# antopio26/quadruped-gym

Hardware: AMD Instinct MI355X
Metric: env_steps_per_sec (higher is better)
Workload: dtype f32

## Files before the change

### quadruped-gym_amd/csrc/qg_kernel_link.hip

```cpp
#define QGK_LINK_ENVS 4
#include "qg_po_dev.h"

typedef const __attribute__((address_space(1))) char *lk_gcbytes;
typedef __attribute__((address_space(1))) char *lk_gbytes;
template <class T> DEV T lk_ld(const T *base, unsigned byte_off) { return *(const __attribute__((address_space(1))) T *)((lk_gcbytes)base + byte_off); }
template <class T> DEV void lk_st(T *base, unsigned byte_off, T v) { *(__attribute__((address_space(1))) T *)((lk_gbytes)base + byte_off) = v; }

template <int CTRL> DEV float dpp_any(float x) {
    return __builtin_bit_cast(float, __builtin_amdgcn_mov_dpp(__builtin_bit_cast(int, x), CTRL, 0xF, 0xF, true));
}
DEV float env_sum(float x) {
#pragma clang fp contract(off)
    x += dpp_any<0xB1>(x);
    x += dpp_any<0x4E>(x);
    x += dpp_any<0x141>(x);
    x += dpp_any<0x140>(x);
    return x;
}
DEV V3 env_sum(V3 a) { return v3(env_sum(a.x), env_sum(a.y), env_sum(a.z)); }
#define QG_T_HM(d, s, bm) "v_add_f32_dpp %[" d "], %[" s "], %[" s "] row_half_mirror row_mask:0xf bank_mask:" bm "\n\t"
#define QG_T_ROR(d, s, bm) "v_add_f32_dpp %[" d "], %[" s "], %[" s "] row_ror:8 row_mask:0xf bank_mask:" bm "\n\t"
#define QG_T_QP(d, qp) "v_add_f32_dpp %[" d "], %[" d "], %[" d "] quad_perm:" qp " row_mask:0xf bank_mask:0xf\n\t"
#define QG_T_L1(g) QG_T_HM("a" g, "a" g, "0x5") QG_T_HM("c" g, "c" g, "0x5") QG_T_HM("a" g, "b" g, "0xa") QG_T_HM("c" g, "d" g, "0xa")
#define QG_T_L2(g) QG_T_ROR("a" g, "a" g, "0x3") QG_T_ROR("a" g, "c" g, "0xc")
#define QG_T_Q1(g) QG_T_QP("a" g, "[1,0,3,2]")
#define QG_T_Q2(g) QG_T_QP("a" g, "[2,3,0,1]")
#define QG_T_OUT(g, v) [a##g] "+v"(v[4 * g]), [c##g] "+v"(v[4 * g + 2])
#define QG_T_IN(g, v) [b##g] "v"(v[4 * g + 1]), [d##g] "v"(v[4 * g + 3])
DEV void env_sum_banked16(float (&v)[16]) {
    asm("s_nop 1\n\t" QG_T_L1("0") QG_T_L1("1") QG_T_L1("2") QG_T_L1("3") QG_T_L2("0") QG_T_L2("1") QG_T_L2("2") QG_T_L2("3")
        QG_T_Q1("0") QG_T_Q1("1") QG_T_Q1("2") QG_T_Q1("3") QG_T_Q2("0") QG_T_Q2("1") QG_T_Q2("2") QG_T_Q2("3") "s_nop 1"
        : QG_T_OUT(0, v), QG_T_OUT(1, v), QG_T_OUT(2, v), QG_T_OUT(3, v)
        : QG_T_IN(0, v), QG_T_IN(1, v), QG_T_IN(2, v), QG_T_IN(3, v));
}
DEV void env_sum_banked12(float (&v)[12]) {
    asm("s_nop 1\n\t" QG_T_L1("0") QG_T_L1("1") QG_T_L1("2") QG_T_L2("0") QG_T_L2("1") QG_T_L2("2")
        QG_T_Q1("0") QG_T_Q1("1") QG_T_Q1("2") QG_T_Q2("0") QG_T_Q2("1") QG_T_Q2("2") "s_nop 1"
        : QG_T_OUT(0, v), QG_T_OUT(1, v), QG_T_OUT(2, v)
        : QG_T_IN(0, v), QG_T_IN(1, v), QG_T_IN(2, v));
}
template <int K> DEV float banked_sum(float r) { return dpp_any<0x150 + 4 * K>(r); }
DEV float leg_suffix(float x) {
#pragma clang fp contract(off)
    x += dpp_any<0xF9>(x);
    x += dpp_any<0xFE>(x);
    return x;
}
DEV float leg_bcast0(float x) { return dpp_any<0x00>(x); }
DEV float leg_bcast1(float x) { return dpp_any<0x55>(x); }
DEV float leg_bcast2(float x) { return dpp_any<0xAA>(x); }

DEV float leg_prefix(float x) {
#pragma clang fp contract(off)
    x += dpp_any<0xD3>(x);
    x += dpp_any<0x4F>(x);
    return x;
}
DEV V3 leg_prefix(V3 a) { return v3(leg_prefix(a.x), leg_prefix(a.y), leg_prefix(a.z)); }

struct LinkRegs {
    float mass, ipos[3], inertia[6], cp[QGK_CP_LINK][3];
    f2 cp2[QGK_CP_LINK / 2][3];
    float lo, hi, damping, armature, kp, kv, gear, force_lo, force_hi, act_decay;
    float cpF[3];
    float ml;
    float fb[8];
};
struct HingeLane { float q, qd, act, u, sn, cs; };
struct KXfrcLink { KWrench w; V3 c0; };

DEV float sel3(int r, float a, float b, float c) { return r == 0 ? a : (r == 1 ? b : c); }
DEV V3 sel3(int r, V3 a, V3 b, V3 c) { return v3(sel3(r, a.x, b.x, c.x), sel3(r, a.y, b.y, c.y), sel3(r, a.z, b.z, c.z)); }

template <bool BAKED, bool DYN = false>
DEV void substep_link(const KModel &C, float cm, float sm, int r, bool lead_env, BaseState &B, HingeLane &J, const LinkRegs &K,
                      bool want_sensors, float *__restrict__ row, int kleg, float &zaxis_z, const KDyn &D = KDyn{}, bool xon = false,
                      const KXfrcLink &X = KXfrcLink{}) {
    using namespace pk3;
    const float h = C.h;
    const BaseCtx bc = pk3::base_prelude_unit(C, B);
    const V3 nb = bc.n;
    if (want_sensors) {
        zaxis_z = bc.cz.z;
        if (r < 3) row[3 * kleg + r] = J.q;
        if (lead_env) {
            row[15] = B.wb.x; row[16] = B.wb.y; row[17] = B.wb.z;
            row[18] = B.pw.x; row[19] = B.pw.y; row[20] = B.pw.z;
            row[21] = B.vw.x; row[22] = B.vw.y; row[23] = B.vw.z;
            row[24] = bc.cx.x; row[25] = bc.cx.y; row[26] = bc.cx.z;
            row[27] = bc.cz.x; row[28] = bc.cz.y; row[29] = bc.cz.z;
            row[30] = bc.vb.x; row[31] = bc.vb.y; row[32] = bc.vb.z;
        }
    }
    const int rr = r < 2 ? r : 2;
    const float snj[3] = {leg_bcast0(J.sn), leg_bcast1(J.sn), leg_bcast2(J.sn)};
    const float csj[3] = {leg_bcast0(J.cs), leg_bcast1(J.cs), leg_bcast2(J.cs)};
    Fr E[3];
    V3 p[3];
    SV S[3];
    {
        Fr Ep = {v3(BAKED ? cm : 1.f, BAKED ? sm : 0.f, 0.f), v3(BAKED ? -sm : 0.f, BAKED ? cm : 1.f, 0.f), v3(0.f, 0.f, 1.f)};
        V3 pp = v3(0.f, 0.f, 0.f);
#pragma unroll
        for (int i = 0; i < 3; ++i) {
            const KLink &L = link_of<BAKED>(C, kleg, i);
            const float sn = snj[i], cs = csj[i];
            p[i] = pp + rot(Ep, ld3(L.pos));
            V3 tx = fma3(L.Q[0], Ep.ex, fma3(L.Q[3], Ep.ey, L.Q[6] * Ep.ez));
            V3 ty = fma3(L.Q[1], Ep.ex, fma3(L.Q[4], Ep.ey, L.Q[7] * Ep.ez));
            V3 tz = fma3(L.Q[2], Ep.ex, fma3(L.Q[5], Ep.ey, L.Q[8] * Ep.ez));
            E[i].ex = fma3(cs, tx, sn * ty);
            E[i].ey = fma3(cs, ty, (-sn) * tx);
            E[i].ez = tz;
// ... 29 lines not shown
        V3 uz = fma3(K.inertia[4], E.ex, fma3(K.inertia[5], E.ey, K.inertia[2] * E.ez));
        float hc = dot(Bi.h, c);
        const f2 uxp = {ux.x, ux.y}, uyp = {uy.x, uy.y}, uzp = {uz.x, uz.y}, hp = {Bi.h.x, Bi.h.y}, cp2 = {c.x, c.y};
        const f2 d2 = __builtin_elementwise_fma(uxp, f2{E.ex.x, E.ex.y}, __builtin_elementwise_fma(uyp, f2{E.ey.x, E.ey.y}, uzp * f2{E.ez.x, E.ez.y}))
                      + f2{hc, hc} - hp * cp2;
        const f2 o2 = __builtin_elementwise_fma(uxp, f2{E.ex.z, E.ex.z}, __builtin_elementwise_fma(uyp, f2{E.ey.z, E.ey.z}, uzp * f2{E.ez.z, E.ez.z}))
                      - hp * f2{c.z, c.z};
        Bi.I.xx = d2.x; Bi.I.yy = d2.y; Bi.I.xz = o2.x; Bi.I.yz = o2.y;
        Bi.I.zz = fmaf(ux.z, E.ex.z, fmaf(uy.z, E.ey.z, uz.z * E.ez.z)) + hc - Bi.h.z * c.z;
        Bi.I.xy = fmaf(ux.x, E.ex.y, fmaf(uy.x, E.ey.y, uz.x * E.ez.y)) - Bi.h.x * c.y;
    }
    SV f;
    {
        SV Iv = mul(Bi, vp), Ia = mul(Bi, ap);
        f.a = cross_add(vp.l, Iv.l, cross_add(vp.a, Iv.a, Ia.a));
        f.l = cross_add(vp.a, Iv.l, Ia.l);
    }
    Sym6 A = sym6_of(Bi);
    {
        const float zo = B.pw.z + dot(nb, pp);
        V3 nl = rotT(Ep, nb);
        float wsum = 0.f;
        V3 s = v3(0.f, 0.f, 0.f);
        const float zb = C.contact_margin - zo;
        if constexpr (BAKED) {
            static_assert(QGK_CP_LINK % 2 == 0, "sample points are taken in pairs");
            f2 w2 = {0.f, 0.f};
            V3T<f2> s2 = v3<f2>(w2, w2, w2);
            const V3T<f2> nl2 = v3<f2>(f2{nl.x, nl.x}, f2{nl.y, nl.y}, f2{nl.z, nl.z});
            const f2 zb2 = {zb, zb};
#pragma unroll
            for (int i = 0; i < QGK_CP_LINK / 2; ++i) contact_point(v3<f2>(K.cp2[i][0], K.cp2[i][1], K.cp2[i][2]), nl2, zb2, w2, s2);
            wsum = w2.x + w2.y;
            s = v3(s2.x.x + s2.x.y, s2.y.x + s2.y.y, s2.z.x + s2.z.y);
        } else {
#pragma unroll
            for (int i = 0; i < QGK_CP_LINK; ++i) contact_point(v3(K.cp[i][0], K.cp[i][1], K.cp[i][2]), nl, zb, wsum, s);
        }
        wsum *= K.ml;
        SV fe;
        ContactDampT<float> cd;
        if constexpr (DYN) pk3::contact_eval(wsum, s, Ep, pp, nb, vp, D.kc, D.cc, C.contact_inv_ramp, D.mu, h, fe, cd);
        else pk3::contact_eval(wsum, s, Ep, pp, nb, vp, C.contact_k, C.contact_c, C.contact_inv_ramp, C.contact_mu, h, fe, cd);
        f.a = f.a - fe.a;
        f.l = f.l - fe.l;
        pk3::add_contact_damping(A, cd.mc, cd.w, cd.P, nb);
    }
    SV xw = {};
    if constexpr (DYN) {
        if (xon) {
            xw = xfrc_spatial(bc, X.w, r < 3 ? cl : X.c0);
            f.a = fma3(-K.ml, xw.a, f.a);
            f.l = fma3(-K.ml, xw.l, f.l);
        }
    }
    float wsumF = 0.f;
    V3 sF = v3(0.f, 0.f, 0.f);
    contact_point(v3(K.cpF[0], K.cpF[1], K.cpF[2]), nb, C.contact_margin - B.pw.z, wsumF, sF);
    wsumF *= K.ml; sF = K.ml * sF;
    Sym6 Ic;
    SV fc;
    Ic.AA.xx = leg_suffix(A.AA.xx); Ic.AA.yy = leg_suffix(A.AA.yy); Ic.AA.zz = leg_suffix(A.AA.zz);
    Ic.AA.xy = leg_suffix(A.AA.xy); Ic.AA.xz = leg_suffix(A.AA.xz); Ic.AA.yz = leg_suffix(A.AA.yz);
    Ic.AL.r0 = v3(leg_suffix(A.AL.r0.x), leg_suffix(A.AL.r0.y), leg_suffix(A.AL.r0.z));
    Ic.AL.r1 = v3(leg_suffix(A.AL.r1.x), leg_suffix(A.AL.r1.y), leg_suffix(A.AL.r1.z));
    Ic.AL.r2 = v3(leg_suffix(A.AL.r2.x), leg_suffix(A.AL.r2.y), leg_suffix(A.AL.r2.z));
    Ic.LL.xx = leg_suffix(A.LL.xx); Ic.LL.yy = leg_suffix(A.LL.yy); Ic.LL.zz = leg_suffix(A.LL.zz);
    Ic.LL.xy = leg_suffix(A.LL.xy); Ic.LL.xz = leg_suffix(A.LL.xz); Ic.LL.yz = leg_suffix(A.LL.yz);
    fc.a = v3(leg_suffix(f.a.x), leg_suffix(f.a.y), leg_suffix(f.a.z));
    fc.l = v3(leg_suffix(f.l.x), leg_suffix(f.l.y), leg_suffix(f.l.z));
    const SV F = mul(Ic, So);
    const float Hc0 = dot(S[0], F), Hc1 = dot(S[1], F);
    const float Hown = dot(So, F);
    const float tb = dot(So, fc);
    float Hd_o, b_o;
    {
        const float q = J.q, qd = J.qd, act = J.act;
        float force = K.kp * (act - K.gear * q) - (K.kv * K.gear) * qd;
        const bool clamped = force <= K.force_lo || force >= K.force_hi;
        force = fminf(fmaxf(force, K.force_lo), K.force_hi);
        float dimp = K.damping + (clamped ? 0.f : K.kv * K.gear * K.gear);
        float tau = K.gear * force - K.damping * qd;
        const float below = K.lo - q, above = q - K.hi;
        const float pen = fmaxf(fmaxf(below, above), 0.f);
        const float bl = C.limit_b * fminf(pen * C.limit_inv_ramp, 1.f);
        const float sg = below > above ? 1.f : -1.f;
        const float sqd = sg * qd;
        const float spring = C.limit_k * pen;
        const float tq = spring - bl * sqd;
        const bool leaving = tq < 0.f;
        tau = fmaf(sg, fmaxf(tq, 0.f), tau);
        dimp = dimp + (leaving ? spring * rcp(sqd) : bl);
        Hd_o = Hown + K.armature + h * dimp;
        b_o = tau - tb;
    }
    const float H00 = leg_bcast0(Hd_o), H01 = leg_bcast1(Hc0), H11 = leg_bcast1(Hd_o);
    const float H02 = leg_bcast2(Hc0), H12 = leg_bcast2(Hc1), H22 = leg_bcast2(Hd_o);
    const float b0 = leg_bcast0(b_o), b1 = leg_bcast1(b_o), b2 = leg_bcast2(b_o);
    const float id0 = rcp(H00);
    const float l10 = H01 * id0, l20 = H02 * id0;
    const float d1 = fmaf(-l10, H01, H11), id1 = rcp(d1);
    const float t21 = fmaf(-l20, H01, H12);
    const float l21 = t21 * id1;
    const float d2 = fmaf(-l21, t21, fmaf(-l20, H02, H22)), id2 = rcp(d2);
    const float y0 = b0, y1 = fmaf(-l10, y0, b1), y2 = fmaf(-l21, y1, fmaf(-l20, y0, b2));
    float z[6] = {F.a.x, F.a.y, F.a.z, F.l.x, F.l.y, F.l.z};
    {
        const float nc0 = r == 1 ? -l10 : (r == 2 ? -l20 : 0.f), nc1 = r == 2 ? -l21 : 0.f;
#pragma unroll
        for (int i = 0; i < 6; ++i) z[i] = fmaf(leg_bcast0(z[i]), nc0, z[i]);
#pragma unroll
        for (int i = 0; i < 6; ++i) z[i] = fmaf(leg_bcast1(z[i]), nc1, z[i]);
    }
    const float idr = sel3(rr, id0, id1, id2), yr = sel3(rr, y0, y1, y2);
    const f2 P = {z[0], z[1]}, L = {z[3], z[4]}, Z = {z[2], z[5]};
    const f2 idr2 = {idr, idr};
    const f2 WP = idr2 * P, WL = idr2 * L, WZ = idr2 * Z;
    Sym6 Cn;
    {
        const f2 Zlo = {Z.x, Z.x}, Zhi = {Z.y, Z.y};
        const f2 WPlo = {WP.x, WP.x}, WPhi = {WP.y, WP.y}, WZlo = {WZ.x, WZ.x};
        const f2 aa0 = __builtin_elementwise_fma(-WP, P, f2{A.AA.xx, A.AA.yy});
        const f2 aa1 = __builtin_elementwise_fma(-WP, Zlo, f2{A.AA.xz, A.AA.yz});
        Cn.AA.xx = aa0.x; Cn.AA.yy = aa0.y; Cn.AA.xz = aa1.x; Cn.AA.yz = aa1.y;
        Cn.AA.xy = fmaf(-WP.x, P.y, A.AA.xy); Cn.AA.zz = fmaf(-WZ.x, Z.x, A.AA.zz);
        const f2 c0 = __builtin_elementwise_fma(-WPlo, L, f2{A.AL.r0.x, A.AL.r0.y});
        const f2 c1 = __builtin_elementwise_fma(-WPhi, L, f2{A.AL.r1.x, A.AL.r1.y});
        const f2 c2 = __builtin_elementwise_fma(-WZlo, L, f2{A.AL.r2.x, A.AL.r2.y});
        const f2 c3 = __builtin_elementwise_fma(-WP, Zhi, f2{A.AL.r0.z, A.AL.r1.z});
        Cn.AL.r0 = v3(c0.x, c0.y, c3.x);
        Cn.AL.r1 = v3(c1.x, c1.y, c3.y);
        Cn.AL.r2 = v3(c2.x, c2.y, fmaf(-WZ.x, Z.y, A.AL.r2.z));
        const f2 l0 = __builtin_elementwise_fma(-WL, L, f2{A.LL.xx, A.LL.yy});
        const f2 l1 = __builtin_elementwise_fma(-WL, Zhi, f2{A.LL.xz, A.LL.yz});
        Cn.LL.xx = l0.x; Cn.LL.yy = l0.y; Cn.LL.xz = l1.x; Cn.LL.yz = l1.y;
        Cn.LL.xy = fmaf(-WL.x, L.y, A.LL.xy); Cn.LL.zz = fmaf(-WZ.y, Z.y, A.LL.zz);
    }
    if constexpr (DYN) {
        if (xon) {
            f.a = fma3(K.ml - 1.f, xw.a, f.a);
            f.l = fma3(K.ml - 1.f, xw.l, f.l);
        }
    }
    const f2 nyr = {-yr, -yr};
    const f2 rh0 = __builtin_elementwise_fma(nyr, WP, f2{-f.a.x, -f.a.y}), rh1 = __builtin_elementwise_fma(nyr, WL, f2{-f.l.x, -f.l.y}),
             rh2 = __builtin_elementwise_fma(nyr, WZ, f2{-f.a.z, -f.l.z});
    SV rhn = {v3(rh0.x, rh0.y, rh2.x), v3(rh1.x, rh1.y, rh2.y)};
    float x6[6];
    {
        SV p0;
        Sym6 Ic0;
        pk3::frame_body_pk<DYN>(C, bc, h, p0, Ic0, D);
        if constexpr (BAKED) {
            Ic0.AA.xx = K.fb[0]; Ic0.AA.yy = K.fb[1]; Ic0.AA.zz = K.fb[2]; Ic0.LL.xx = K.fb[3]; Ic0.LL.yy = K.fb[4]; Ic0.LL.zz = K.fb[5];
            Ic0.AL.r0.y = K.fb[6]; Ic0.AL.r1.x = K.fb[7];
        }
        float t16[16] = {Cn.AA.xx, Cn.AA.yy, Cn.AA.zz, Cn.AA.xy, Cn.AA.xz, Cn.AA.yz, Cn.AL.r0.x, Cn.AL.r0.y,
                         Cn.AL.r0.z, Cn.AL.r1.x, Cn.AL.r1.y, Cn.AL.r1.z, Cn.AL.r2.x, Cn.AL.r2.y, Cn.AL.r2.z, wsumF};
        float t12[12] = {Cn.LL.xx, Cn.LL.yy, Cn.LL.zz, Cn.LL.xy, Cn.LL.xz, Cn.LL.yz, rhn.a.x, rhn.a.y, rhn.a.z, rhn.l.x, rhn.l.y, rhn.l.z};
        env_sum_banked16(t16);
        env_sum_banked12(t12);
        Ic0.AA.xx += banked_sum<0>(t16[0]); Ic0.AA.yy += banked_sum<1>(t16[0]); Ic0.AA.zz += banked_sum<2>(t16[0]); Ic0.AA.xy += banked_sum<3>(t16[0]);
        Ic0.AA.xz += banked_sum<0>(t16[4]); Ic0.AA.yz += banked_sum<1>(t16[4]); Ic0.AL.r0.x += banked_sum<2>(t16[4]); Ic0.AL.r0.y += banked_sum<3>(t16[4]);
        Ic0.AL.r0.z += banked_sum<0>(t16[8]); Ic0.AL.r1.x += banked_sum<1>(t16[8]); Ic0.AL.r1.y += banked_sum<2>(t16[8]); Ic0.AL.r1.z += banked_sum<3>(t16[8]);
        Ic0.AL.r2.x += banked_sum<0>(t16[12]); Ic0.AL.r2.y += banked_sum<1>(t16[12]); Ic0.AL.r2.z += banked_sum<2>(t16[12]);
        wsumF = banked_sum<3>(t16[12]);
        Ic0.LL.xx += banked_sum<0>(t12[0]); Ic0.LL.yy += banked_sum<1>(t12[0]); Ic0.LL.zz += banked_sum<2>(t12[0]); Ic0.LL.xy += banked_sum<3>(t12[0]);
        Ic0.LL.xz += banked_sum<0>(t12[4]); Ic0.LL.yz += banked_sum<1>(t12[4]);
        SV b = {v3(banked_sum<2>(t12[4]) - p0.a.x, banked_sum<3>(t12[4]) - p0.a.y, banked_sum<0>(t12[8]) - p0.a.z),
                v3(banked_sum<1>(t12[8]) - p0.l.x, banked_sum<2>(t12[8]) - p0.l.y, banked_sum<3>(t12[8]) - p0.l.z)};
        if (__any(wsumF > 0.f)) {
            sF = env_sum(sF);
            Fr E0 = {v3(1.f, 0.f, 0.f), v3(0.f, 1.f, 0.f), v3(0.f, 0.f, 1.f)};
            SV fe;
            if constexpr (DYN) contact_finish(wsumF, sF, E0, v3(0.f, 0.f, 0.f), bc.n, bc.V0, D.kc, D.cc, C.contact_inv_ramp, D.mu, h, fe, Ic0);
            else contact_finish(wsumF, sF, E0, v3(0.f, 0.f, 0.f), bc.n, bc.V0, C.contact_k, C.contact_c, C.contact_inv_ramp, C.contact_mu, h, fe, Ic0);
            b.a = b.a + fe.a;
            b.l = b.l + fe.l;
        }
        pk3::base_solve(Ic0, b, x6);
    }
    const V3 wdot = v3(x6[0], x6[1], x6[2]);
    const V3 acl = v3(x6[3], x6[4], x6[5]);
    if (want_sensors && lead_env) {
        row[12] = acl.x - bc.gb.x; row[13] = acl.y - bc.gb.y; row[14] = acl.z - bc.gb.z;
    }
    {
        const float g_o = fmaf(F.a.x, x6[0], fmaf(F.a.y, x6[1], fmaf(F.a.z, x6[2], fmaf(F.l.x, x6[3], fmaf(F.l.y, x6[4], F.l.z * x6[5])))));
        const float r0 = b0 - leg_bcast0(g_o), r1 = b1 - leg_bcast1(g_o), r2 = b2 - leg_bcast2(g_o);
        const float yy0 = r0, yy1 = fmaf(-l10, yy0, r1), yy2 = fmaf(-l21, yy1, fmaf(-l20, yy0, r2));
        const float qdd2 = yy2 * id2;
        const float qdd1 = fmaf(-l21, qdd2, yy1 * id1);
        const float qdd0 = fmaf(-l20, qdd2, fmaf(-l10, qdd1, yy0 * id0));
        J.qd = fmaf(h, sel3(rr, qdd0, qdd1, qdd2), J.qd);
        J.q = fmaf(h, J.qd, J.q);
        hinge_advance(h * J.qd, J.sn, J.cs);
        J.act = fmaf(J.u - J.act, K.act_decay, J.act);
    }
    pk3::base_integrate_unit(bc, h, wdot, acl, B);
}

#define QGK_LINK_WAVES 4
template <bool WALK = false, bool PO = false, bool BAKED = true, bool HELP = false, bool DYN = false>
__global__ __launch_bounds__(QGK_WAVE * QGK_LINK_WAVES * (HELP ? 2 : 1), 1) void qg_step_kernel_link(const KModel *__restrict__ Mp, const KTask *__restrict__ T, KStepArgs P,
                                                                                  const typename WalkArgT<WALK>::type WK,
                                                                                  const typename PoArgT<PO>::type PK) {
    static_assert(WALK || !PO, "the observation pack rides on the walking task layer");
    static_assert(WALK || !HELP, "the helper waves carry the walking task layer's estimator");
    static_assert(!DYN || (!BAKED && !HELP), "per-env dynamics: the table-driven variants");
    static_assert(QGK_LINK_ENVS * QGK_LINK_WAVES == QG_PO_ENVS && QGK_WAVE * QGK_LINK_WAVES == QG_PO_THREADS, "workgroup layout of qg_po_dev.h");
    __shared__ float tile_all[QGK_LINK_WAVES][QGK_LINK_ENVS * 35];
    __shared__ KModel smodel;
    QG_STAGE_MODEL(C, BAKED, smodel, Mp, QGK_WAVE * QGK_LINK_WAVES * (HELP ? 2 : 1));
    QG_TASK_REGS(Tk, T);
    QG_MARK(0);
    const int lane = threadIdx.x & (QGK_WAVE - 1);
    const int wave = (threadIdx.x >> 6) & (QGK_LINK_WAVES - 1);
    const bool helper = HELP && (threadIdx.x >> 6) >= QGK_LINK_WAVES;
    float *tile = tile_all[wave];
    const int r = lane & 3;
    const int k = (lane >> 2) & 3;
    const int el = lane >> 4;
    const int env0 = (blockIdx.x * QGK_LINK_WAVES + wave) * QGK_LINK_ENVS;
    const int n = P.n;
    const bool live = env0 + el < n;
    const int env = live ? env0 + el : n - 1;
    const bool lead_env = (lane & 15) == 0;
    const float cm = (k == 0) ? 1.f : (k == 2) ? -1.f : 0.f;
    const float sm = (k == 1) ? 1.f : (k == 3) ? -1.f : 0.f;

    constexpr bool RWDH = HELP && !PO;
    __shared__ float s_est[HELP ? QGK_LINK_WAVES : 1][QGK_WAVE][2];
// ... 150 lines not shown
            if constexpr (!HELP) walk_estimator_finish_n<1>(WK.P, WK.S, n, tt, xx, calls, west, wf, wa);
            WK.S.eff_actions[(size_t)env * 12 + jch] = a_eff;
        }
    }
    PoHistRegs phist = {};
    if constexpr (PO) {
        int slot = pin.head + 1;
        if (slot >= PK.P.window) slot = 0;
        if (!HELP && PK.P.window > 1) po_copy_history_load(PK.P, PK.S, (size_t)env * (PK.P.window * QG_PO_FRAME), slot, lane & 15, PK.out, live, phist);
    }

    float *srow = tile + el * 35;
    float zaxis_z = 1.f;
    const int fs = Tk.frame_skip;
    if constexpr (BAKED && !PO && HELP == WALK) __builtin_assume(fs >= 1);
#ifdef QG_PHASE_TIMES
    asm volatile("" :: "v"(B.pw.x), "v"(B.qw), "v"(B.vw.x), "v"(B.wb.x), "v"(J.q), "v"(J.qd), "v"(J.act), "v"(J.sn), "v"(J.cs));
#endif
    QG_MARK(1);
    asm volatile(".p2align 6");
#pragma unroll 1
    for (int s = 0; s < fs; ++s) substep_link<BAKED, DYN>(C, cm, sm, r, lead_env, B, J, K, s == fs - 1, srow, k, zaxis_z, D, xon, X);
    int nstep = nstep0 + fs;
    QG_MARK(2);

    const float ssq = env_sum(r < 3 ? aclip * aclip : 0.f);
    QG_REWARD_TERMS(Tk., B, ssq, nstep);
    QG_DONE_IF_BAD_STATE(B, env_sum(r < 3 ? J.q + J.qd : 0.f));
    const int od = Tk.obs_mode == 1 ? 21 : 33;
    const int row = P.packed ? od + 2 : od;
    QG_DONE_IF_FLIPPED(Tk., zaxis_z);
    const bool lead = live && lead_env;
    const bool rst = done && Tk.auto_reset;
    if (rst) QG_BASE_RESET(B, nstep, C.qpos0, Tk., P, env, P.st.episode[env]);
    if constexpr (HELP) {
        if constexpr (PO) {
            const int le = 4 * wave + el;
            if (wch) s_new[le][11 + jch] = aclip;
            if (lead_env) {
                s_hand[le][0] = done ? 1.f : 0.f;
                s_hand[le][1] = B.qw; s_hand[le][2] = B.qx; s_hand[le][3] = B.qy; s_hand[le][4] = B.qz;
            }
        }
        if constexpr (RWDH) {
            if (lead_env) {
                s_done[wave][el] = done ? 1.f : 0.f;
                if (od == 21) { srow[18] = srow[30]; srow[19] = srow[31]; srow[20] = srow[32]; }
            }
        }
        __syncthreads();
        if constexpr (!RWDH) {
            wf[0] = s_est[wave][lane][0];
            wa[0] = s_est[wave][lane][1];
        }
    }
    if (lead) {
        QG_BASE_STORE(B, nstep, P.st, QG_PUT_LK, n4, e4);
        if (rst) P.st.episode[env] += 1;
    }
    if (wch) {
        const float q0 = BAKED ? sel3(rk, C.qpos0[7], C.qpos0[8], C.qpos0[9]) : C.qpos0[7 + jch];
        const unsigned j4 = (unsigned)jch * n4 + e4;
        lk_st(P.st.qpos, 7 * n4 + j4, rst ? q0 : J.q);
        lk_st(P.st.qvel, 6 * n4 + j4, rst ? 0.f : J.qd);
        lk_st(P.st.act, j4, rst ? 0.f : J.act);
        if (P.track_ctrl) lk_st(P.st.ctrl, j4, rst ? Tk.default_ctrl[jch] : aclip);
    }
    if (lead_env) {
        if (!RWDH && od == 21) { srow[18] = srow[30]; srow[19] = srow[31]; srow[20] = srow[32]; }
        if (P.packed) { srow[od] = reward; srow[od + 1] = done ? 1.f : 0.f; }
    }
    wave_sync();
    if constexpr (!PO) {
        const int live_envs = max(0, min(QGK_LINK_ENVS, n - env0));
        const int total = live_envs * row;
        float *dst = (P.packed ? P.packed : P.obs) + (size_t)env0 * row;
        if (row == 35) {
            float v[3];
#pragma unroll
            for (int u = 0; u < 3; ++u) v[u] = tile[min(lane + u * QGK_WAVE, QGK_LINK_ENVS * 35 - 1)];
#pragma unroll
            for (int u = 0; u < 3; ++u) if (lane + u * QGK_WAVE < total) dst[lane + u * QGK_WAVE] = v[u];
        } else {
            float v[QGK_LINK_ENVS];
#pragma unroll
            for (int er = 0; er < QGK_LINK_ENVS; ++er) v[er] = tile[er * 35 + min(lane, 34)];
#pragma unroll
            for (int er = 0; er < QGK_LINK_ENVS; ++er) if (er < live_envs && lane < row) dst[er * row + lane] = v[er];
        }
    }
    QG_MARK(3);
    if (lead && !P.packed) {
        if constexpr (!WALK) P.reward[env] = reward;
        P.done[env] = done ? 1 : 0;
    }
    if constexpr (WALK && !RWDH) {
        WalkSums sum = {0.f, 0.f, 0.f, 0.f};
        if (wch) {
            walk_channel_terms(WK.S, env, jch, wtg, aclip, wprev, wf[0], wa[0], sum);
// ... 31 lines not shown
```

### quadruped-gym_amd/csrc/qg_kernels.hip

```cpp
#include <hip/hip_runtime.h>
#include <stdint.h>

#include "qg_device.h"
#include "qg_model_baked.h"
#include "qg_step_shell.h"

#define DEV __device__ __forceinline__
#define QG_STR2(x) #x
#define QG_STR(x) QG_STR2(x)

static __device__ const KModel QG_BAKED_MODEL = {QG_BAKED_FLOATS};
template <bool BAKED> DEV const KModel &table(const KModel *__restrict__ M) {
    if constexpr (BAKED) return QG_BAKED_MODEL; else return *M;
}
template <bool BAKED> DEV const KLink &link_of(const KModel &C, int k, int i) { return C.link[BAKED ? i : 3 * k + i]; }

typedef float f2 __attribute__((ext_vector_type(2)));
typedef int i2 __attribute__((ext_vector_type(2)));

DEV float fma_(float a, float b, float c) { return fmaf(a, b, c); }
DEV f2 fma_(f2 a, f2 b, f2 c) { return __builtin_elementwise_fma(a, b, c); }
DEV float max_(float a, float b) { return fmaxf(a, b); }
DEV f2 max_(f2 a, f2 b) { f2 r = {fmaxf(a.x, b.x), fmaxf(a.y, b.y)}; return r; }
DEV float min_(float a, float b) { return fminf(a, b); }
// ... 17 lines not shown
template <class T> DEV T splat(float x) { return T(x); }

template <class T> struct V3T { T x, y, z; };
typedef V3T<float> V3;
template <class T> DEV V3T<T> v3(T x, T y, T z) { V3T<T> r = {x, y, z}; return r; }
template <class T> DEV V3T<T> operator+(V3T<T> a, V3T<T> b) { return v3<T>(a.x + b.x, a.y + b.y, a.z + b.z); }
template <class T> DEV V3T<T> operator-(V3T<T> a, V3T<T> b) { return v3<T>(a.x - b.x, a.y - b.y, a.z - b.z); }
template <class T> DEV V3T<T> operator*(T s, V3T<T> a) { return v3<T>(s * a.x, s * a.y, s * a.z); }
template <class T> DEV T dot(V3T<T> a, V3T<T> b) { return fma_(a.x, b.x, fma_(a.y, b.y, a.z * b.z)); }
template <class T> DEV V3T<T> cross(V3T<T> a, V3T<T> b) { return v3<T>(a.y * b.z - a.z * b.y, a.z * b.x - a.x * b.z, a.x * b.y - a.y * b.x); }
template <class T> DEV V3T<T> fma3(T s, V3T<T> a, V3T<T> b) { return v3<T>(fma_(s, a.x, b.x), fma_(s, a.y, b.y), fma_(s, a.z, b.z)); }
namespace pk3 {
DEV V3 fma3(float s, V3 a, V3 b) { f2 A = {a.x, a.y}, Bv = {b.x, b.y}, S = {s, s}; f2 r = __builtin_elementwise_fma(S, A, Bv); return v3<float>(r.x, r.y, fmaf(s, a.z, b.z)); }
DEV V3 operator+(V3 a, V3 b) { f2 A = {a.x, a.y}, Bv = {b.x, b.y}; f2 r = A + Bv; return v3<float>(r.x, r.y, a.z + b.z); }
DEV V3 operator-(V3 a, V3 b) { f2 A = {a.x, a.y}, Bv = {b.x, b.y}; f2 r = A - Bv; return v3<float>(r.x, r.y, a.z - b.z); }
DEV V3 operator*(float s, V3 a) { f2 A = {a.x, a.y}, S = {s, s}; f2 r = S * A; return v3<float>(r.x, r.y, s * a.z); }
DEV bool has_literal(V3 a) { return __builtin_constant_p(a.x) || __builtin_constant_p(a.y) || __builtin_constant_p(a.z); }
DEV V3 cross(V3 a, V3 b) {
    if (has_literal(a) || has_literal(b)) return ::cross<float>(a, b);
    f2 A = {a.x, a.y}, Bv = {b.x, b.y}, az, bz, m, r;
    az.x = a.z; bz.x = b.z;
    asm("v_pk_mul_f32 %0, %1, %2 op_sel:[0,1] op_sel_hi:[0,0] neg_lo:[1,0]" : "=v"(m) : "v"(az), "v"(Bv));
    asm("v_pk_fma_f32 %0, %1, %2, %3 op_sel:[1,0,0] op_sel_hi:[0,0,1] neg_hi:[1,0,0]" : "=v"(r) : "v"(A), "v"(bz), "v"(m));
    return v3<float>(r.x, r.y, a.x * b.y - a.y * b.x);
}
DEV V3 cross_add(V3 a, V3 b, V3 acc) {
    if (has_literal(a) || has_literal(b)) return ::operator+<float>(acc, ::cross<float>(a, b));
    f2 A = {a.x, a.y}, Bv = {b.x, b.y}, C2 = {acc.x, acc.y}, az, bz, m, r;
    az.x = a.z; bz.x = b.z;
    asm("v_pk_fma_f32 %0, %1, %2, %3 op_sel:[0,1,0] op_sel_hi:[0,0,1] neg_lo:[1,0,0]" : "=v"(m) : "v"(az), "v"(Bv), "v"(C2));
    asm("v_pk_fma_f32 %0, %1, %2, %3 op_sel:[1,0,0] op_sel_hi:[0,0,1] neg_hi:[1,0,0]" : "=v"(r) : "v"(A), "v"(bz), "v"(m));
    return v3<float>(r.x, r.y, fmaf(a.x, b.y, fmaf(-a.y, b.x, acc.z)));
}
}
DEV V3 ld3(const float *p) { return v3<float>(p[0], p[1], p[2]); }
template <class T> DEV V3T<T> ld3t(const float *p) { return v3<T>(T(p[0]), T(p[1]), T(p[2])); }
template <class T> DEV V3T<T> splat3(V3 a) { return v3<T>(T(a.x), T(a.y), T(a.z)); }

template <class T> struct FrT { V3T<T> ex, ey, ez; };
typedef FrT<float> Fr;
template <class T> DEV V3T<T> rot(const FrT<T> &E, V3T<T> r) { return fma3(r.x, E.ex, fma3(r.y, E.ey, r.z * E.ez)); }
template <class T> DEV V3T<T> rotT(const FrT<T> &E, V3T<T> r) { return v3<T>(dot(E.ex, r), dot(E.ey, r), dot(E.ez, r)); }

template <class T> struct Sym3T { T xx, yy, zz, xy, xz, yz; };
typedef Sym3T<float> Sym3;
template <class T> DEV V3T<T> mul(const Sym3T<T> &S, V3T<T> v) {
    return v3<T>(fma_(S.xx, v.x, fma_(S.xy, v.y, S.xz * v.z)), fma_(S.xy, v.x, fma_(S.yy, v.y, S.yz * v.z)),
                 fma_(S.xz, v.x, fma_(S.yz, v.y, S.zz * v.z)));
}
template <class T> DEV void add(Sym3T<T> &a, const Sym3T<T> &b) { a.xx += b.xx; a.yy += b.yy; a.zz += b.zz; a.xy += b.xy; a.xz += b.xz; a.yz += b.yz; }
template <class T> DEV void rank1(Sym3T<T> &a, T w, V3T<T> u, V3T<T> v) {
    a.xx = fma_(w * u.x, v.x, a.xx); a.yy = fma_(w * u.y, v.y, a.yy); a.zz = fma_(w * u.z, v.z, a.zz);
    a.xy = fma_(w * u.x, v.y, a.xy); a.xz = fma_(w * u.x, v.z, a.xz); a.yz = fma_(w * u.y, v.z, a.yz);
}

template <class T> struct M3T { V3T<T> r0, r1, r2; };
typedef M3T<float> M3;
template <class T> DEV V3T<T> mul(const M3T<T> &A, V3T<T> v) { return v3<T>(dot(A.r0, v), dot(A.r1, v), dot(A.r2, v)); }
template <class T> DEV V3T<T> mulT(const M3T<T> &A, V3T<T> v) { return fma3(v.x, A.r0, fma3(v.y, A.r1, v.z * A.r2)); }
template <class T> DEV void add(M3T<T> &a, const M3T<T> &b) { a.r0 = a.r0 + b.r0; a.r1 = a.r1 + b.r1; a.r2 = a.r2 + b.r2; }

template <class T> struct SVT { V3T<T> a, l; };
typedef SVT<float> SV;
template <class T> DEV SVT<T> operator+(SVT<T> p, SVT<T> q) { SVT<T> r = {p.a + q.a, p.l + q.l}; return r; }
template <class T> DEV T dot(SVT<T> p, SVT<T> q) { return dot(p.a, q.a) + dot(p.l, q.l); }
template <class T> DEV SVT<T> splat6(SV v) { SVT<T> r = {splat3<T>(v.a), splat3<T>(v.l)}; return r; }
// ... 144 lines not shown

DEV void wave_sync() {
    __builtin_amdgcn_fence(__ATOMIC_RELEASE, "wavefront");
    __builtin_amdgcn_wave_barrier();
    __builtin_amdgcn_fence(__ATOMIC_ACQUIRE, "wavefront");
}

#include "qg_walk_dev.h"
#include "qg_po_dev.h"

DEV float jittered_hinge(float q0, float lo, float hi, float jitter, uint64_t seed, uint64_t env_index, int episode, int j) {
    float u = uniform24s(seed, env_index, (uint64_t)episode, QG_STREAM_HINGE + (uint32_t)j);
    return fminf(fmaxf(fmaf(jitter, 2.f * u - 1.f, q0), lo), hi);
}

template <class T> DEV void contact_point(V3T<T> r, V3T<T> nl, T zb, T &wsum, V3T<T> &s) {
    T pen = max_(fma_(-nl.x, r.x, fma_(-nl.y, r.y, fma_(-nl.z, r.z, zb))), T(0.f));
    wsum += pen;
    s = fma3(pen, r, s);
}
template <class T> struct ContactDampT { T mc, w; V3T<T> P; };
#define QG_TEMPLATE_T template <class T>
#define QG_CROSS_ADD(a, b, acc) ((acc) + cross((a), (b)))
#include "qg_contact_eval.inc"
#undef QG_CROSS_ADD
#undef QG_TEMPLATE_T
namespace pk3 {
typedef float T;
#define QG_TEMPLATE_T
#define QG_CROSS_ADD(a, b, acc) cross_add((a), (b), (acc))
#include "qg_contact_eval.inc"
#undef QG_CROSS_ADD
#undef QG_TEMPLATE_T
DEV void add_contact_damping(Sym6 &A, float m, float w, V3 r, V3 n) {
    const float rr = dot(r, r);
    const V3 h = m * r;
    const f2 hxy = {h.x, h.y}, rxy = {r.x, r.y}, nxy = {n.x, n.y};
    const float mrr = m * rr;
    const f2 aad = f2{A.AA.xx, A.AA.yy} + __builtin_elementwise_fma(-hxy, rxy, f2{mrr, mrr});
    const f2 aao = __builtin_elementwise_fma(-hxy, f2{r.z, r.z}, f2{A.AA.xz, A.AA.yz});
    A.AA.zz += fmaf(-h.z, r.z, mrr);
    A.AA.xy = fmaf(-h.x, r.y, A.AA.xy);
    A.AL.r0.y -= h.z; A.AL.r0.z += h.y;
    A.AL.r1.x += h.z; A.AL.r1.z -= h.x;
    const f2 r2xy = f2{A.AL.r2.x, A.AL.r2.y} + f2{-h.y, h.x};
    const f2 lld = f2{A.LL.xx, A.LL.yy} + f2{m, m};
    A.LL.zz += m;
    const V3 ra = cross(r, n), wra = w * ra, wn = w * n;
    const f2 raxy = {ra.x, ra.y}, wraxy = {wra.x, wra.y}, wnxy = {wn.x, wn.y};
    const f2 aad2 = __builtin_elementwise_fma(wraxy, raxy, aad);
    const f2 aao2 = __builtin_elementwise_fma(wraxy, f2{ra.z, ra.z}, aao);
    A.AA.xx = aad2.x; A.AA.yy = aad2.y; A.AA.xz = aao2.x; A.AA.yz = aao2.y;
    A.AA.xy = fmaf(wra.x, ra.y, A.AA.xy); A.AA.zz = fmaf(wra.z, ra.z, A.AA.zz);
    A.AL.r0 = fma3(wra.x, n, A.AL.r0);
    A.AL.r1 = fma3(wra.y, n, A.AL.r1);
    A.AL.r2 = fma3(wra.z, n, v3<float>(r2xy.x, r2xy.y, A.AL.r2.z));
    const f2 lld2 = __builtin_elementwise_fma(wnxy, nxy, lld);
    const f2 llo = __builtin_elementwise_fma(wnxy, f2{n.z, n.z}, f2{A.LL.xz, A.LL.yz});
    A.LL.xx = lld2.x; A.LL.yy = lld2.y; A.LL.xz = llo.x; A.LL.yz = llo.y;
    A.LL.xy = fmaf(wn.x, n.y, A.LL.xy); A.LL.zz = fmaf(wn.z, n.z, A.LL.zz);
}
}
template <class T>
DEV void contact_finish(T wsum, V3T<T> s, const FrT<T> &E, V3T<T> p, V3T<T> n, SVT<T> v, float kc, float cmax, float inv_ramp, float mu, float h,
                        SVT<T> &f_ext, Sym6T<T> &A) {
    ContactDampT<T> cd;
    contact_eval(wsum, s, E, p, n, v, kc, cmax, inv_ramp, mu, h, f_ext, cd);
    add_contact_damping(A, cd.mc, cd.w, cd.P, n);
}
template <class T, int NCP>
DEV void contact_points(const float (*cp)[3], V3T<T> nl, T zb, T &wsum, V3T<T> &s) {
    wsum = T(0.f);
    s = v3<T>(T(0.f), T(0.f), T(0.f));
#pragma unroll
    for (int i = 0; i < NCP; ++i) contact_point(ld3t<T>(cp[i]), nl, zb, wsum, s);
}
template <class T, int NCP>
DEV void body_contact(const float (*cp)[3], const FrT<T> &E, V3T<T> p, T z_origin, V3T<T> n, SVT<T> v, float kc, float cmax, float inv_ramp,
                      float margin, float mu, float h, SVT<T> &f_ext, Sym6T<T> &A) {
    V3T<T> nl = rotT(E, n);
    T wsum;
    V3T<T> s;
    contact_points<T, NCP>(cp, nl, T(margin) - z_origin, wsum, s);
    contact_finish(wsum, s, E, p, n, v, kc, cmax, inv_ramp, mu, h, f_ext, A);
}
template <class T, int NCP>
DEV void body_contact_compact(const float (*cp)[3], const FrT<T> &E, V3T<T> p, T z_origin, V3T<T> n, SVT<T> v, float kc, float cmax, float inv_ramp,
// ... 452 lines not shown
}

template <bool RSQ = false>
DEV void base_integrate(const BaseCtx &c, float h, V3 wdot, V3 acl, BaseState &B) {
    V3 aw = fma3(acl.x, c.cx, fma3(acl.y, c.cy, acl.z * c.cz));
    B.vw = fma3(h, aw, B.vw);
    B.wb = fma3(h, wdot, B.wb);
    B.pw = fma3(h, B.vw, B.pw);
    float hh = 0.5f * h;
    float x2 = hh * hh * dot(B.wb, B.wb);
    float sc, cw;
    if constexpr (RSQ) {
        sc = hh * fmaf(x2, fmaf(x2, 1.f / 120.f, -1.f / 6.f), 1.f);
        cw = fmaf(x2, fmaf(x2, 1.f / 24.f, -0.5f), 1.f);
    } else {
        sc = hh * fmaf(x2, fmaf(x2, fmaf(x2, -1.f / 5040.f, 1.f / 120.f), -1.f / 6.f), 1.f);
        cw = fmaf(x2, fmaf(x2, fmaf(x2, -1.f / 720.f, 1.f / 24.f), -0.5f), 1.f);
    }
    V3 dv = sc * B.wb;
    float w = c.w, x = c.x, y = c.y, z = c.z;
    float nw = w * cw - x * dv.x - y * dv.y - z * dv.z;
    float nx = w * dv.x + x * cw + y * dv.z - z * dv.y;
    float ny = w * dv.y - x * dv.z + y * cw + z * dv.x;
    float nz = w * dv.z + x * dv.y - y * dv.x + z * cw;
    const float n2 = nw * nw + nx * nx + ny * ny + nz * nz;
    float inv = RSQ ? __builtin_amdgcn_rsqf(n2) : rcp(__builtin_amdgcn_sqrtf(n2));
    B.qw = nw * inv; B.qx = nx * inv; B.qy = ny * inv; B.qz = nz * inv;
}

namespace pk3 {
#define QG_PKFMA(dst, a, b, c, MODS) asm("v_pk_fma_f32 %0, %1, %2, %3 " MODS : "=v"(dst) : "v"(a), "v"(b), "v"(c))
#define QG_PKMUL(dst, a, b, MODS) asm("v_pk_mul_f32 %0, %1, %2 " MODS : "=v"(dst) : "v"(a), "v"(b))
DEV float opaque(float v) { asm("" : "+v"(v)); return v; }
DEV BaseCtx base_prelude_unit(const KModel &C, const BaseState &B) {
    BaseCtx c;
    const f2 W = {B.qw, B.qz}, X = {opaque(B.qx), opaque(B.qy)};
    const f2 W2 = W + W, X2 = X + X;
    const f2 m10 = {-1.f, 0.f};
    f2 A, cxp, cyp, T, czp, np;
    QG_PKFMA(A, W2, W, m10, "op_sel_hi:[0,1,1]");
    QG_PKFMA(cxp, X2, X, A, "op_sel_hi:[0,1,1]");
    QG_PKFMA(cyp, X2, X, A, "op_sel:[1,0,1] op_sel_hi:[1,1,0] neg_lo:[0,0,1]");
    QG_PKMUL(T, W2, X, "op_sel:[0,1] op_sel_hi:[0,0]");
    QG_PKFMA(czp, X2, W, T, "op_sel:[0,1,0] op_sel_hi:[1,1,1] neg_hi:[0,0,1]");
    QG_PKFMA(np, X2, W, T, "op_sel:[0,1,0] op_sel_hi:[1,1,1] neg_lo:[0,0,1]");
    c.cx = v3(cxp.x, cxp.y, np.x);
    c.cy = v3(cyp.x, cyp.y, np.y);
    c.cz = v3(czp.x, czp.y, fmaf(W2.y, W.y, A.x));
    c.n = v3(c.cx.z, c.cy.z, c.cz.z);
    V3 gw = ld3(C.g);
    c.gb = v3(dot(c.cx, gw), dot(c.cy, gw), dot(c.cz, gw));
    c.vb = v3(dot(c.cx, B.vw), dot(c.cy, B.vw), dot(c.cz, B.vw));
    c.V0.a = B.wb; c.V0.l = c.vb;
    c.A0.a = v3(0.f, 0.f, 0.f);
    c.A0.l = cross_add(c.vb, B.wb, v3(-c.gb.x, -c.gb.y, -c.gb.z));
    return c;
}
DEV void base_integrate_unit(const BaseCtx &c, float h, V3 wdot, V3 acl, BaseState &B) {
    V3 aw = fma3(acl.x, c.cx, fma3(acl.y, c.cy, acl.z * c.cz));
    B.vw = fma3(h, aw, B.vw);
    B.wb = fma3(h, wdot, B.wb);
    B.pw = fma3(h, B.vw, B.pw);
    const float hh = 0.5f * h;
    const float x2 = hh * hh * dot(B.wb, B.wb);
    const float sc = hh * fmaf(x2, fmaf(x2, 1.f / 120.f, -1.f / 6.f), 1.f);
    const float cw = fmaf(x2, fmaf(x2, 1.f / 24.f, -0.5f), 1.f);
    const V3 dv = sc * B.wb;
    const f2 W = {B.qw, B.qz}, X = {opaque(B.qx), opaque(B.qy)};
    const f2 DW = {cw, dv.z}, DX = {dv.x, dv.y};
    f2 a, b;
    QG_PKMUL(a, W, DW, "op_sel:[1,1] op_sel_hi:[1,0] neg_lo:[0,1]");
    QG_PKFMA(a, X, DX, a, "op_sel:[1,1,0] op_sel_hi:[1,0,1] neg_lo:[0,1,0] neg_hi:[0,1,0]");
    QG_PKFMA(a, X, DX, a, "op_sel_hi:[0,1,1] neg_lo:[0,1,0]");
    QG_PKFMA(a, W, DW, a, "op_sel_hi:[0,1,1]");
    QG_PKMUL(b, W, DX, "op_sel:[1,1] op_sel_hi:[1,0] neg_lo:[0,1]");
    QG_PKFMA(b, X, DW, b, "op_sel:[1,1,0] op_sel_hi:[1,0,1]");
    QG_PKFMA(b, X, DW, b, "op_sel_hi:[0,1,1] neg_hi:[0,1,0]");
    QG_PKFMA(b, W, DX, b, "op_sel_hi:[0,1,1]");
    const f2 n2 = __builtin_elementwise_fma(b, b, a * a);
    const float inv = __builtin_amdgcn_rsqf(n2.x + n2.y);
    const f2 i2 = {inv, inv};
    a = a * i2; b = b * i2;
    B.qw = a.x; B.qz = a.y; B.qx = b.x; B.qy = b.y;
}
#undef QG_PKFMA
#undef QG_PKMUL
}

#define LQ(j) (0 + (j))
#define LQD(j) (12 + (j))
#define LACT(j) (24 + (j))
#define LU(j) (36 + (j))
#define LY(k, i) (48 + 21 * (k) + (i))
#define QG_LDS_SLOTS (48 + 21 * 4)
#define QG_OBS_TILE_FLOATS (64 * 35)

struct SensorOut { float accel[3]; V3 pw, vw, wb, vb, xaxis, zaxis; };

template <bool BAKED>
DEV void substep(const KModel *__restrict__ Mp, float *__restrict__ lds, int lane, BaseState &B, bool want_sensors, SensorOut &so,
                 float *__restrict__ jpos_out) {
// ... 1014 lines not shown
```

Baseline: 422.3 million.

## Micro-optimise baked link substep with packed and DPP-fused instructions

In the baked link kernel path, the leg-1 broadcast followed by an FMA is folded into a single v_fmac_f32_dpp per element. The quaternion x/y values are carried through the base context into the integrate step, and gravity subtraction uses a dedicated packed cross_sub. Contact damping gains a rigid variant that builds the angular-linear block entries from Bi.h with packed add/fma, instead of doing scalar updates. Smaller tweaks add opaque barriers in the contact sum, hoist the default-ctrl load ahead of the reset, and make the episode increment atomic. The aim is to trim VALU instruction count and register moves, at the cost of more inline assembly that relies on exact DPP and op_sel semantics.

```diff
diff --git a/quadruped-gym_amd/csrc/qg_kernel_link.hip b/quadruped-gym_amd/csrc/qg_kernel_link.hip
--- a/quadruped-gym_amd/csrc/qg_kernel_link.hip
+++ b/quadruped-gym_amd/csrc/qg_kernel_link.hip
@@ -46,6 +46,7 @@
     x += dpp_any<0xFE>(x);
     return x;
 }
+#define QG_Z_FM(i) "v_fmac_f32_dpp %[z" i "], %[z" i "], %[c] quad_perm:[1,1,1,1] row_mask:0xf bank_mask:0xf\n\t"
 DEV float leg_bcast0(float x) { return dpp_any<0x00>(x); }
 DEV float leg_bcast1(float x) { return dpp_any<0x55>(x); }
 DEV float leg_bcast2(float x) { return dpp_any<0xAA>(x); }
@@ -78,7 +79,7 @@
                       const KXfrcLink &X = KXfrcLink{}) {
     using namespace pk3;
     const float h = C.h;
-    const BaseCtx bc = pk3::base_prelude_unit(C, B);
+    const BaseCtx bc = pk3::base_prelude_unit<BAKED>(C, B);
     const V3 nb = bc.n;
     if (want_sensors) {
         zaxis_z = bc.cz.z;
@@ -174,7 +175,7 @@
 #pragma unroll
             for (int i = 0; i < QGK_CP_LINK / 2; ++i) contact_point(v3<f2>(K.cp2[i][0], K.cp2[i][1], K.cp2[i][2]), nl2, zb2, w2, s2);
             wsum = w2.x + w2.y;
-            s = v3(s2.x.x + s2.x.y, s2.y.x + s2.y.y, s2.z.x + s2.z.y);
+            s = v3(opaque(s2.x.x + s2.x.y), opaque(s2.y.x + s2.y.y), s2.z.x + s2.z.y);
         } else {
 #pragma unroll
             for (int i = 0; i < QGK_CP_LINK; ++i) contact_point(v3(K.cp[i][0], K.cp[i][1], K.cp[i][2]), nl, zb, wsum, s);
@@ -186,7 +187,8 @@
         else pk3::contact_eval(wsum, s, Ep, pp, nb, vp, C.contact_k, C.contact_c, C.contact_inv_ramp, C.contact_mu, h, fe, cd);
         f.a = f.a - fe.a;
         f.l = f.l - fe.l;
-        pk3::add_contact_damping(A, cd.mc, cd.w, cd.P, nb);
+        if constexpr (BAKED) pk3::add_contact_damping<true>(A, cd.mc, cd.w, cd.P, nb, Bi.h);
+        else pk3::add_contact_damping(A, cd.mc, cd.w, cd.P, nb);
     }
     SV xw = {};
     if constexpr (DYN) {
@@ -251,8 +253,14 @@
         const float nc0 = r == 1 ? -l10 : (r == 2 ? -l20 : 0.f), nc1 = r == 2 ? -l21 : 0.f;
 #pragma unroll
         for (int i = 0; i < 6; ++i) z[i] = fmaf(leg_bcast0(z[i]), nc0, z[i]);
-#pragma unroll
-        for (int i = 0; i < 6; ++i) z[i] = fmaf(leg_bcast1(z[i]), nc1, z[i]);
+        if constexpr (BAKED) {
+            asm("s_nop 1\n\t" QG_Z_FM("0") QG_Z_FM("1") QG_Z_FM("2") QG_Z_FM("3") QG_Z_FM("4") QG_Z_FM("5")
+                : [z0] "+v"(z[0]), [z1] "+v"(z[1]), [z2] "+v"(z[2]), [z3] "+v"(z[3]), [z4] "+v"(z[4]), [z5] "+v"(z[5])
+                : [c] "v"(nc1));
+        } else {
+#pragma unroll
+            for (int i = 0; i < 6; ++i) z[i] = fmaf(leg_bcast1(z[i]), nc1, z[i]);
+        }
     }
     const float idr = sel3(rr, id0, id1, id2), yr = sel3(rr, y0, y1, y2);
     const f2 P = {z[0], z[1]}, L = {z[3], z[4]}, Z = {z[2], z[5]};
@@ -286,7 +294,8 @@
     }
     const f2 nyr = {-yr, -yr};
     const f2 rh0 = __builtin_elementwise_fma(nyr, WP, f2{-f.a.x, -f.a.y}), rh1 = __builtin_elementwise_fma(nyr, WL, f2{-f.l.x, -f.l.y}),
-             rh2 = __builtin_elementwise_fma(nyr, WZ, f2{-f.a.z, -f.l.z});
+             rh2 = BAKED ? __builtin_elementwise_fma(nyr, WZ, -f2{f.a.z, f.l.z})
+                         : __builtin_elementwise_fma(nyr, WZ, f2{-f.a.z, -f.l.z});
     SV rhn = {v3(rh0.x, rh0.y, rh2.x), v3(rh1.x, rh1.y, rh2.y)};
     float x6[6];
     {
@@ -339,7 +348,7 @@
         hinge_advance(h * J.qd, J.sn, J.cs);
         J.act = fmaf(J.u - J.act, K.act_decay, J.act);
     }
-    pk3::base_integrate_unit(bc, h, wdot, acl, B);
+    pk3::base_integrate_unit<BAKED>(bc, h, wdot, acl, B);
 }
 
 #define QGK_LINK_WAVES 4
@@ -556,7 +565,11 @@
     QG_DONE_IF_FLIPPED(Tk., zaxis_z);
     const bool lead = live && lead_env;
     const bool rst = done && Tk.auto_reset;
-    if (rst) QG_BASE_RESET(B, nstep, C.qpos0, Tk., P, env, P.st.episode[env]);
+    float ctrl0 = 0.f;
+    if (rst) {
+        ctrl0 = Tk.default_ctrl[jch];
+        QG_BASE_RESET(B, nstep, C.qpos0, Tk., P, env, P.st.episode[env]);
+    }
     if constexpr (HELP) {
         if constexpr (PO) {
             const int le = 4 * wave + el;
@@ -580,7 +593,7 @@
     }
     if (lead) {
         QG_BASE_STORE(B, nstep, P.st, QG_PUT_LK, n4, e4);
-        if (rst) P.st.episode[env] += 1;
+        if (rst) __hip_atomic_fetch_add(P.st.episode + env, 1, __ATOMIC_RELAXED, __HIP_MEMORY_SCOPE_AGENT);
     }
     if (wch) {
         const float q0 = BAKED ? sel3(rk, C.qpos0[7], C.qpos0[8], C.qpos0[9]) : C.qpos0[7 + jch];
@@ -588,7 +601,7 @@
         lk_st(P.st.qpos, 7 * n4 + j4, rst ? q0 : J.q);
         lk_st(P.st.qvel, 6 * n4 + j4, rst ? 0.f : J.qd);
         lk_st(P.st.act, j4, rst ? 0.f : J.act);
-        if (P.track_ctrl) lk_st(P.st.ctrl, j4, rst ? Tk.default_ctrl[jch] : aclip);
+        if (P.track_ctrl) lk_st(P.st.ctrl, j4, rst ? ctrl0 : aclip);
     }
     if (lead_env) {
         if (!RWDH && od == 21) { srow[18] = srow[30]; srow[19] = srow[31]; srow[20] = srow[32]; }
diff --git a/quadruped-gym_amd/csrc/qg_kernels.hip b/quadruped-gym_amd/csrc/qg_kernels.hip
--- a/quadruped-gym_amd/csrc/qg_kernels.hip
+++ b/quadruped-gym_amd/csrc/qg_kernels.hip
@@ -73,6 +73,14 @@
     asm("v_pk_fma_f32 %0, %1, %2, %3 op_sel:[1,0,0] op_sel_hi:[0,0,1] neg_hi:[1,0,0]" : "=v"(r) : "v"(A), "v"(bz), "v"(m));
     return v3<float>(r.x, r.y, fmaf(a.x, b.y, fmaf(-a.y, b.x, acc.z)));
 }
+DEV V3 cross_sub(V3 a, V3 b, V3 acc) {
+    if (has_literal(a) || has_literal(b)) return cross_add(a, b, v3<float>(-acc.x, -acc.y, -acc.z));
+    f2 A = {a.x, a.y}, Bv = {b.x, b.y}, C2 = {acc.x, acc.y}, az, bz, m, r;
+    az.x = a.z; bz.x = b.z;
+    asm("v_pk_fma_f32 %0, %1, %2, %3 op_sel:[0,1,0] op_sel_hi:[0,0,1] neg_lo:[1,0,1] neg_hi:[0,0,1]" : "=v"(m) : "v"(az), "v"(Bv), "v"(C2));
+    asm("v_pk_fma_f32 %0, %1, %2, %3 op_sel:[1,0,0] op_sel_hi:[0,0,1] neg_hi:[1,0,0]" : "=v"(r) : "v"(A), "v"(bz), "v"(m));
+    return v3<float>(r.x, r.y, fmaf(a.x, b.y, fmaf(-a.y, b.x, -acc.z)));
+}
 }
 DEV V3 ld3(const float *p) { return v3<float>(p[0], p[1], p[2]); }
 template <class T> DEV V3T<T> ld3t(const float *p) { return v3<T>(T(p[0]), T(p[1]), T(p[2])); }
@@ -283,7 +291,8 @@
 #include "qg_contact_eval.inc"
 #undef QG_CROSS_ADD
 #undef QG_TEMPLATE_T
-DEV void add_contact_damping(Sym6 &A, float m, float w, V3 r, V3 n) {
+template <bool RIGID = false>
+DEV void add_contact_damping(Sym6 &A, float m, float w, V3 r, V3 n, V3 bh = V3{}) {
     const float rr = dot(r, r);
     const V3 h = m * r;
     const f2 hxy = {h.x, h.y}, rxy = {r.x, r.y}, nxy = {n.x, n.y};
@@ -292,9 +301,15 @@
     const f2 aao = __builtin_elementwise_fma(-hxy, f2{r.z, r.z}, f2{A.AA.xz, A.AA.yz});
     A.AA.zz += fmaf(-h.z, r.z, mrr);
     A.AA.xy = fmaf(-h.x, r.y, A.AA.xy);
-    A.AL.r0.y -= h.z; A.AL.r0.z += h.y;
+    A.AL.r0.z += h.y;
     A.AL.r1.x += h.z; A.AL.r1.z -= h.x;
-    const f2 r2xy = f2{A.AL.r2.x, A.AL.r2.y} + f2{-h.y, h.x};
+    f2 r2xy;
+    if constexpr (RIGID) {
+        asm("v_pk_add_f32 %0, %1, %2 op_sel:[1,1] op_sel_hi:[0,0] neg_lo:[1,1]" : "=v"(r2xy) : "v"(f2{bh.x, bh.y}), "v"(hxy));
+    } else {
+        A.AL.r0.y -= h.z;
+        r2xy = f2{A.AL.r2.x, A.AL.r2.y} + f2{-h.y, h.x};
+    }
     const f2 lld = f2{A.LL.xx, A.LL.yy} + f2{m, m};
     A.LL.zz += m;
     const V3 ra = cross(r, n), wra = w * ra, wn = w * n;
@@ -303,7 +318,14 @@
     const f2 aao2 = __builtin_elementwise_fma(wraxy, f2{ra.z, ra.z}, aao);
     A.AA.xx = aad2.x; A.AA.yy = aad2.y; A.AA.xz = aao2.x; A.AA.yz = aao2.y;
     A.AA.xy = fmaf(wra.x, ra.y, A.AA.xy); A.AA.zz = fmaf(wra.z, ra.z, A.AA.zz);
-    A.AL.r0 = fma3(wra.x, n, A.AL.r0);
+    if constexpr (RIGID) {
+        const f2 r1xy = {A.AL.r1.x, A.AL.r1.y};
+        f2 r0xy;
+        asm("v_pk_fma_f32 %0, %1, %2, %3 op_sel:[0,0,1] op_sel_hi:[0,1,0] neg_hi:[0,0,1]" : "=v"(r0xy) : "v"(wraxy), "v"(nxy), "v"(r1xy));
+        A.AL.r0 = v3<float>(r0xy.x, r0xy.y, fmaf(wra.x, n.z, A.AL.r0.z));
+    } else {
+        A.AL.r0 = fma3(wra.x, n, A.AL.r0);
+    }
     A.AL.r1 = fma3(wra.y, n, A.AL.r1);
     A.AL.r2 = fma3(wra.z, n, v3<float>(r2xy.x, r2xy.y, A.AL.r2.z));
     const f2 lld2 = __builtin_elementwise_fma(wnxy, nxy, lld);
@@ -822,9 +844,11 @@
 #define QG_PKFMA(dst, a, b, c, MODS) asm("v_pk_fma_f32 %0, %1, %2, %3 " MODS : "=v"(dst) : "v"(a), "v"(b), "v"(c))
 #define QG_PKMUL(dst, a, b, MODS) asm("v_pk_mul_f32 %0, %1, %2 " MODS : "=v"(dst) : "v"(a), "v"(b))
 DEV float opaque(float v) { asm("" : "+v"(v)); return v; }
+template <bool CARRY = false>
 DEV BaseCtx base_prelude_unit(const KModel &C, const BaseState &B) {
     BaseCtx c;
     const f2 W = {B.qw, B.qz}, X = {opaque(B.qx), opaque(B.qy)};
+    if constexpr (CARRY) { c.x = X.x; c.y = X.y; }
     const f2 W2 = W + W, X2 = X + X;
     const f2 m10 = {-1.f, 0.f};
     f2 A, cxp, cyp, T, czp, np;
@@ -843,9 +867,11 @@
     c.vb = v3(dot(c.cx, B.vw), dot(c.cy, B.vw), dot(c.cz, B.vw));
     c.V0.a = B.wb; c.V0.l = c.vb;
     c.A0.a = v3(0.f, 0.f, 0.f);
-    c.A0.l = cross_add(c.vb, B.wb, v3(-c.gb.x, -c.gb.y, -c.gb.z));
+    if constexpr (CARRY) c.A0.l = cross_sub(c.vb, B.wb, c.gb);
+    else c.A0.l = cross_add(c.vb, B.wb, v3(-c.gb.x, -c.gb.y, -c.gb.z));
     return c;
 }
+template <bool CARRY = false>
 DEV void base_integrate_unit(const BaseCtx &c, float h, V3 wdot, V3 acl, BaseState &B) {
     V3 aw = fma3(acl.x, c.cx, fma3(acl.y, c.cy, acl.z * c.cz));
     B.vw = fma3(h, aw, B.vw);
@@ -856,7 +882,10 @@
     const float sc = hh * fmaf(x2, fmaf(x2, 1.f / 120.f, -1.f / 6.f), 1.f);
     const float cw = fmaf(x2, fmaf(x2, 1.f / 24.f, -0.5f), 1.f);
     const V3 dv = sc * B.wb;
-    const f2 W = {B.qw, B.qz}, X = {opaque(B.qx), opaque(B.qy)};
+    f2 X;
+    if constexpr (CARRY) X = f2{c.x, c.y};
+    else X = f2{opaque(B.qx), opaque(B.qy)};
+    const f2 W = {B.qw, B.qz};
     const f2 DW = {cw, dv.z}, DX = {dv.x, dv.y};
     f2 a, b;
     QG_PKMUL(a, W, DW, "op_sel:[1,1] op_sel_hi:[1,0] neg_lo:[0,1]");
```

After: 427.7 million, median of 6. 1.3% higher.
